# X-PLUG/Youku-mPLUG

Hardware: NVIDIA H100
Metric: video-text samples/sec (pretrain 1.3B, 8f x 224^2) (higher is better)
Workload: dtype bf16

## Files before the change

youku-mplug_b200/csrc/attention.cu:

```cuda
#include <math_constants.h>
#include <stdlib.h>

#include "common.h"
#include "philox.cuh"
#include "ptx.cuh"
#include "wgmma.cuh"

namespace ymp {

struct SeqMap {
  int seq_div, n_prefix, prefix_per_seq;
  long outer_stride, inner_stride, pos_stride, prefix_base, prefix_stride;
};
static SeqMap to_map(const ymp_seqmap& m) {
  SeqMap r;
  r.seq_div = m.seq_div > 0 ? m.seq_div : 1;
  r.n_prefix = m.n_prefix; r.prefix_per_seq = m.prefix_per_seq;
  r.outer_stride = m.outer_stride; r.inner_stride = m.inner_stride; r.pos_stride = m.pos_stride;
  r.prefix_base = m.prefix_base; r.prefix_stride = m.prefix_stride;
  return r;
}
struct RSeq {
  long base, pos_stride, prefix0;
  int n_prefix;
// ... 72 lines not shown
  a = w0 >= ds.thresh ? a * ds.scale : 0.f;
  b = w1 >= ds.thresh ? b * ds.scale : 0.f;
}
__device__ __forceinline__ float drop1(const DropState& ds, uint32_t row, uint32_t col, float a) {
  const uint4 w = drop_words(ds, row, col >> 2);
  const uint32_t c = col & 3, wc = c == 0 ? w.x : c == 1 ? w.y : c == 2 ? w.z : w.w;
  return wc >= ds.thresh ? a * ds.scale : 0.f;
}

__device__ __forceinline__ void eff_len(const AttnKParams& p, int s, int& sq, int& skv) {
  sq = p.s_q; skv = p.s_kv;
  if (p.skv_dev) skv = min(skv, *p.skv_dev);
  if (p.total_rows > 0) {
    const long left = p.total_rows - (long)s * p.s_q;
    if (left < sq) sq = (int)left;
    if (left < skv) skv = (int)left;
  }
}
__device__ __forceinline__ bool tile_needs_mask(const AttnKParams& p, int row_lo, int col0, int skv) {
  if (col0 + 64 > skv) return true;
  if (p.mask == MASK_CAUSAL) return col0 + 63 > row_lo;
  return p.mask == MASK_BLOCK;
}
__device__ __forceinline__ void apply_mask(const AttnKParams& p, float (&sc)[8][4], int row_lo, int col0, int skv,
                                           int g, int t4, float fill) {
  const int r0 = row_lo + g, r1 = r0 + 8;
  int rb0 = 0, rb1 = 0;
  if (p.mask == MASK_BLOCK) { rb0 = r0 / p.mask_block; rb1 = r1 / p.mask_block; }
#pragma unroll
  for (int nb = 0; nb < 8; ++nb) {
#pragma unroll
    for (int e = 0; e < 2; ++e) {
      const int col = col0 + nb * 8 + t4 * 2 + e;
      bool m0 = col >= skv, m1 = m0;
      if (p.mask == MASK_CAUSAL) { m0 |= col > r0; m1 |= col > r1; }
      else if (p.mask == MASK_BLOCK) { const int cb = col / p.mask_block; m0 |= cb != rb0; m1 |= cb != rb1; }
      if (m0) sc[nb][e] = fill;
      if (m1) sc[nb][2 + e] = fill;
    }
  }
}
template <bool BLOCK>
__device__ __forceinline__ void apply_mask_t(const AttnKParams& p, float (&st)[8][4], int k_lo, int qi0, int skv, int g,
                                             int t4) {
  bool need = k_lo + 16 > skv;
  if (p.mask == MASK_CAUSAL) need |= k_lo + 15 > qi0;
  if (BLOCK && p.mask == MASK_BLOCK) need = true;
  if (!need) return;
  const int k0 = k_lo + g, k1 = k0 + 8;
  int kb0 = 0, kb1 = 0;
  if (BLOCK && p.mask == MASK_BLOCK) { kb0 = k0 / p.mask_block; kb1 = k1 / p.mask_block; }
#pragma unroll
  for (int nb = 0; nb < 8; ++nb) {
#pragma unroll
    for (int e = 0; e < 2; ++e) {
      const int qc = qi0 + nb * 8 + t4 * 2 + e;
      bool m0 = k0 >= skv, m1 = k1 >= skv;
      if (p.mask == MASK_CAUSAL) { m0 |= k0 > qc; m1 |= k1 > qc; }
      else if (BLOCK && p.mask == MASK_BLOCK) { const int qb = qc / p.mask_block; m0 |= qb != kb0; m1 |= qb != kb1; }
      if (m0) st[nb][e] = -CUDART_INF_F;
      if (m1) st[nb][2 + e] = -CUDART_INF_F;
    }
  }
}

template <bool BLOCK>
__device__ __forceinline__ int key_tiles(const AttnKParams& p, int a_lo, int sq, int skv, int& kv_begin) {
  int kv_end = skv;
  kv_begin = 0;
  if (p.mask == MASK_CAUSAL) kv_end = min(skv, a_lo + 64);
  if (BLOCK && p.mask == MASK_BLOCK) {
    kv_begin = (a_lo / p.mask_block) * p.mask_block / 64 * 64;
    kv_end = min(skv, ((min(a_lo + 64, sq) - 1) / p.mask_block + 1) * p.mask_block);
  }
  return (kv_end - kv_begin + 63) / 64;
}
__device__ __forceinline__ void warp_key_span(const AttnKParams& p, int r_lo, int kv0, int skv, int& nv, int& nb_lo) {
  nv = min(64, skv - kv0);
  nb_lo = 0;
  if (p.mask == MASK_CAUSAL) nv = min(nv, r_lo + 16 - kv0);
  if (p.mask == MASK_BLOCK) {
    const int c_lo = (r_lo / p.mask_block) * p.mask_block, c_hi = ((r_lo + 15) / p.mask_block + 1) * p.mask_block;
    nb_lo = max(0, (c_lo - kv0) / 16);
    nv = min(nv, c_hi - kv0);
  }
}

template <int ND>
__device__ __forceinline__ void softmax_step(const AttnKParams& p, float (&sc)[8][4], float (&m_i)[2], float (&l_i)[2],
                                             float (&o_acc)[ND][4]) {
  float mx[2] = {-CUDART_INF_F, -CUDART_INF_F};
#pragma unroll
  for (int nb = 0; nb < 8; ++nb) {
    mx[0] = fmaxf(mx[0], fmaxf(sc[nb][0], sc[nb][1]));
    mx[1] = fmaxf(mx[1], fmaxf(sc[nb][2], sc[nb][3]));
  }
  float alpha[2], ms[2];
#pragma unroll
  for (int r = 0; r < 2; ++r) {
    mx[r] = fmaxf(mx[r], __shfl_xor_sync(0xffffffffu, mx[r], 1));
    mx[r] = fmaxf(mx[r], __shfl_xor_sync(0xffffffffu, mx[r], 2));
    const float mnew = fmaxf(m_i[r], mx[r]);
    ms[r] = (mnew == -CUDART_INF_F) ? 0.f : mnew * p.scale_log2;
    alpha[r] = exp2f(m_i[r] * p.scale_log2 - ms[r]);
    m_i[r] = mnew;
    l_i[r] *= alpha[r];
  }
#pragma unroll
  for (int nb = 0; nb < 8; ++nb) {
#pragma unroll
    for (int e = 0; e < 4; ++e) {
      const float pv = exp2f(fmaf(sc[nb][e], p.scale_log2, -ms[e >> 1]));
      sc[nb][e] = pv;
      l_i[e >> 1] += pv;
    }
  }
#pragma unroll
  for (int i = 0; i < ND; ++i) {
    o_acc[i][0] *= alpha[0]; o_acc[i][1] *= alpha[0];
    o_acc[i][2] *= alpha[1]; o_acc[i][3] *= alpha[1];
  }
}
__device__ __forceinline__ void drop_tile(const DropState& ds, uint32_t drow0, int kv0, int t4, float (&f)[8][4]) {
#pragma unroll
  for (int nb = 0; nb < 8; ++nb) {
    const uint32_t col = (uint32_t)(kv0 + nb * 8 + t4 * 2);
    drop2(ds, drow0, col, f[nb][0], f[nb][1]);
    drop2(ds, drow0 + 8, col, f[nb][2], f[nb][3]);
  }
}
__device__ __forceinline__ void scores_to_ds(const AttnKParams& p, float (&sc)[8][4], const float (&dp)[8][4],
                                             const float (&lse_r)[2], const float (&del_r)[2]) {
#pragma unroll
  for (int nb = 0; nb < 8; ++nb) {
#pragma unroll
    for (int e = 0; e < 4; ++e) {
      const float pv = exp2f(fmaf(sc[nb][e], p.scale_log2, -lse_r[e >> 1]));
      sc[nb][e] = pv * (dp[nb][e] - del_r[e >> 1]);
    }
  }
}
template <bool QUAD_EXCHANGE>
__device__ __forceinline__ void probs_t(const AttnKParams& p, const DropState& ds, float (&st)[8][4], float (&dpt)[8][4],
                                        const float* stat, uint32_t qrow0, int k_lo, int lane) {
  const int g = lane >> 2, t4 = lane & 3;
#pragma unroll
  for (int nb = 0; nb < 8; ++nb) {
    uint32_t keep = 0xFu;
    if (QUAD_EXCHANGE && p.has_drop) {
      const int j = g & 3;
      const uint32_t qr = qrow0 + (uint32_t)(nb * 8 + t4 * 2 + (j & 1));
      const uint4 w = drop_words(ds, qr, (uint32_t)(k_lo + (g & ~3) + (j >> 1) * 8) >> 2);
      keep = 0;
#pragma unroll
      for (int r = 0; r < 4; ++r) {
        const int comp = (j + r) & 3, c = (j - r) & 3;
        const uint32_t v = comp == 0 ? w.x : comp == 1 ? w.y : comp == 2 ? w.z : w.w;
        const uint32_t got = __shfl_sync(0xffffffffu, v, (lane & ~0xC) | (c << 2));
        keep |= (got >= ds.thresh ? 1u : 0u) << c;
      }
    }
#pragma unroll
    for (int e = 0; e < 4; ++e) {
      const int ql = nb * 8 + t4 * 2 + (e & 1);
      const float pv = exp2f(fmaf(st[nb][e], p.scale_log2, -stat[ql]));
      float dz = dpt[nb][e];
      if (p.has_drop) {
        float kf;
        if constexpr (QUAD_EXCHANGE) {
          kf = (keep >> e) & 1u ? ds.scale : 0.f;
// ... 460 lines not shown
      }
    }
    __syncthreads();
  }
  if (!warp_active) return;
  store_dkdv<D, DIO>(p, dk_acc, dv_acc, kv0 + warp * 16, skv, h, mdkv, g, t4);
}

template <int D>
struct WgTile {
  static constexpr int BYTES = ((D + 63) / 64) * 8192;
};
__device__ __forceinline__ uint64_t wg_desc_k(uint32_t base, int ks) {
  return make_smem_desc(base + (ks >> 2) * 8192 + (ks & 3) * 32, 16, 1024, 1);
}
__device__ __forceinline__ uint64_t wg_desc_mn(uint32_t base, int ks) { return make_smem_desc(base + ks * 2048, 8192, 1024, 1); }

template <int D>
__device__ __forceinline__ void wg_rs(float (&d)[D / 2], const uint32_t (&a)[4], uint64_t db) {
  if constexpr (D == 64) wgmma_rs_m64n64_tb(d, a, db);
  else if constexpr (D == 80) wgmma_rs_m64n80_tb(d, a, db);
  else wgmma_rs_m64n96_tb(d, a, db);
}
template <int D>
__device__ __forceinline__ void wg_scores(float (&s)[8][4], uint32_t a, uint32_t b) {
  float (&f)[32] = *reinterpret_cast<float(*)[32]>(&s[0][0]);
#pragma unroll
  for (int i = 0; i < 32; ++i) f[i] = 0.f;
  wgmma_fence_acc(f);
  wgmma_fence();
#pragma unroll
  for (int kk = 0; kk < D / 16; ++kk) wgmma_ss_m64n64(f, wg_desc_k(a, kk), wg_desc_k(b, kk));
  wgmma_commit();
  wgmma_wait<0>();
  wgmma_fence_acc(f);
}
template <int D>
__device__ __forceinline__ void wg_pv(float (&acc)[D / 8][4], const float (&pm)[8][4], uint32_t t) {
  float (&f)[D / 2] = *reinterpret_cast<float(*)[D / 2]>(&acc[0][0]);
  uint32_t pa[4][4];
#pragma unroll
  for (int kk = 0; kk < 4; ++kk) {
    pa[kk][0] = pack_bf16(pm[2 * kk][0], pm[2 * kk][1]);
    pa[kk][1] = pack_bf16(pm[2 * kk][2], pm[2 * kk][3]);
    pa[kk][2] = pack_bf16(pm[2 * kk + 1][0], pm[2 * kk + 1][1]);
    pa[kk][3] = pack_bf16(pm[2 * kk + 1][2], pm[2 * kk + 1][3]);
  }
  wgmma_fence_acc(f);
  wgmma_fence();
#pragma unroll
  for (int kk = 0; kk < 4; ++kk) wg_rs<D>(f, pa[kk], wg_desc_mn(t, kk));
  wgmma_commit();
  wgmma_wait<0>();
  wgmma_fence_acc(f);
}

template <bool CACHE>
__device__ __forceinline__ auto with_cache(const RMat& m, const __nv_bfloat16* c, const AttnKParams& p, int s, int h) {
  if constexpr (CACHE) return RMatC{m, c + (long)(s / p.mkv.seq_div) * p.n0 * p.ldc + h * p.hsc, p.ldc, p.n0};
  else return m;
}

template <bool PACKED>
__device__ __forceinline__ RSeq seq_rows(const SeqMap& m, int s, int r0) {
  if constexpr (PACKED) return RSeq{r0, 1, 0, 0};
  else return resolve(m, s);
}

template <int D, int DIO, bool TABLE = false, bool CACHE = false, bool PACKED = false>
__global__ void __launch_bounds__(128) attn_wg_fwd_kernel(const AttnKParams p) {
  constexpr int TB = WgTile<D>::BYTES;
  extern __shared__ uint8_t smem_wg[];
  uint8_t* sm = smem_wg + ((1024u - (smem_u32(smem_wg) & 1023u)) & 1023u);
  uint8_t* Qs = sm;
  uint8_t* KVs = sm + TB;
  const int warp = threadIdx.x >> 5, lane = threadIdx.x & 31;
  const int h = blockIdx.y, s = blockIdx.z;
  const int g = lane >> 2, t4 = lane & 3;
  int qoff = p.mask == MASK_CAUSAL ? p.s_kv - p.s_q : 0;
  int q0 = blockIdx.x * 64 - (qoff & 63), a0 = q0 + qoff;
  if constexpr (TABLE) {
    qoff = __ldg(p.n_prefix + s / p.mkv.seq_div);
    q0 = blockIdx.x * 64 - (qoff & 63);
    a0 = q0 + qoff;
  }
  int sq, skv;
  eff_len(p, s, sq, skv);
  if constexpr (TABLE) skv = qoff + sq;
  int r0 = 0;
  if constexpr (PACKED) {
    r0 = __ldg(p.starts + s);
    sq = skv = __ldg(p.starts + s + 1) - r0;
  }
  if (q0 >= sq) return;
  RSeq mkv = seq_rows<PACKED>(p.mkv, s, r0);
  const RSeq mo = seq_rows<PACKED>(p.mo, s, r0);
  if constexpr (TABLE) mkv.n_prefix = CACHE ? qoff - p.n0 : qoff;
  const RMat Mq = rmat(p.q, seq_rows<PACKED>(p.mq, s, r0), p.ldq, h * p.hsq);
  const auto Mk = with_cache<CACHE>(rmat(p.k, mkv, p.ldk, h * p.hsk), p.kc, p, s, h);
  const auto Mv = with_cache<CACHE>(rmat(p.v, mkv, p.ldv, h * p.hsv), p.vc, p, s, h);
  int kv_begin;
  const int ntiles = key_tiles<false>(p, a0, sq, skv, kv_begin);

  load_tile<SWIZZLE_128B, D, DIO>(Qs, Mq, q0, sq);
  load_tile<SWIZZLE_128B, D, DIO>(KVs, Mk, kv_begin, skv);
  load_tile<SWIZZLE_128B, D, DIO>(KVs + TB, Mv, kv_begin, skv);
  cp_async_commit();

  float o_acc[D / 8][4];
#pragma unroll
  for (int i = 0; i < D / 8; ++i) { o_acc[i][0] = o_acc[i][1] = o_acc[i][2] = o_acc[i][3] = 0.f; }
  float m_i[2] = {-CUDART_INF_F, -CUDART_INF_F}, l_i[2] = {0.f, 0.f};
  DropState ds;
  if (p.has_drop) ds = drop_state(p.drop);
  const uint32_t drow0 = (uint32_t)(((long)s * p.n_heads + h) * p.s_q + q0 + warp * 16 + g);

  for (int t = 0; t < ntiles; ++t) {
    const int kv0 = kv_begin + t * 64;
    uint8_t* Ks = KVs + (t & 1) * 2 * TB;
    uint8_t* Vs = Ks + TB;
    if (t + 1 < ntiles) {
      uint8_t* Kn = KVs + ((t + 1) & 1) * 2 * TB;
      load_tile<SWIZZLE_128B, D, DIO>(Kn, Mk, kv0 + 64, skv);
      load_tile<SWIZZLE_128B, D, DIO>(Kn + TB, Mv, kv0 + 64, skv);
      cp_async_commit();
      cp_async_wait<1>();
    } else {
      cp_async_wait<0>();
    }
    fence_proxy_async();
    __syncthreads();
    float sc[8][4];
    wg_scores<D>(sc, smem_u32(Qs), smem_u32(Ks));
    if (tile_needs_mask(p, a0 + warp * 16, kv0, skv)) apply_mask(p, sc, a0 + warp * 16, kv0, skv, g, t4, -CUDART_INF_F);
    softmax_step(p, sc, m_i, l_i, o_acc);
    if (p.has_drop) drop_tile(ds, drow0, kv0, t4, sc);
    wg_pv<D>(o_acc, sc, smem_u32(Vs));
    __syncthreads();
  }
  store_o_lse<D, DIO, PACKED>(p, o_acc, m_i, l_i, q0 + warp * 16, sq, s, h, mo, g, t4);
}

template <int D, int DIO>
__global__ void __launch_bounds__(128) attn_wg_bwd_dq_kernel(const AttnKParams p) {
  constexpr int TB = WgTile<D>::BYTES;
  extern __shared__ uint8_t smem_wg[];
  uint8_t* sm = smem_wg + ((1024u - (smem_u32(smem_wg) & 1023u)) & 1023u);
  uint8_t* Qs = sm;
  uint8_t* dOs = sm + TB;
  uint8_t* KVs = sm + 2 * TB;
  float* stat = reinterpret_cast<float*>(sm + 6 * TB);
  const int warp = threadIdx.x >> 5, lane = threadIdx.x & 31;
  const int q0 = blockIdx.x * 64, h = blockIdx.y, s = blockIdx.z;
  const int g = lane >> 2, t4 = lane & 3;
  int sq, skv;
  eff_len(p, s, sq, skv);
  if (q0 >= sq) return;
  const RSeq mkv = resolve(p.mkv, s), mo = resolve(p.mo, s), mdo = resolve(p.mdo, s), mdq = resolve(p.mdq, s);
  const RMat Mq = rmat(p.q, resolve(p.mq, s), p.ldq, h * p.hsq), Mdo = rmat(p.dout, mdo, p.lddo, h * p.hsdo);
  const RMat Mk = rmat(p.k, mkv, p.ldk, h * p.hsk), Mv = rmat(p.v, mkv, p.ldv, h * p.hsv);
  int kv_begin;
  const int ntiles = key_tiles<false>(p, q0, sq, skv, kv_begin);

  load_tile<SWIZZLE_128B, D, DIO>(Qs, Mq, q0, sq);
  load_tile<SWIZZLE_128B, D, DIO>(dOs, Mdo, q0, sq);
  load_tile<SWIZZLE_128B, D, DIO>(KVs, Mk, kv_begin, skv);
  load_tile<SWIZZLE_128B, D, DIO>(KVs + TB, Mv, kv_begin, skv);
  cp_async_commit();
  stage_dq_stats<DIO>(p, s, h, q0 + warp * 16, sq, mo, mdo, stat + warp * 16);
  float dq_acc[D / 8][4];
#pragma unroll
  for (int i = 0; i < D / 8; ++i) { dq_acc[i][0] = dq_acc[i][1] = dq_acc[i][2] = dq_acc[i][3] = 0.f; }
  float lse_r[2], del_r[2];
  DropState ds;
  if (p.has_drop) ds = drop_state(p.drop);
  const uint32_t drow0 = (uint32_t)(((long)s * p.n_heads + h) * p.s_q + q0 + warp * 16 + g);

  for (int t = 0; t < ntiles; ++t) {
    const int kv0 = kv_begin + t * 64;
    uint8_t* Ks = KVs + (t & 1) * 2 * TB;
    uint8_t* Vs = Ks + TB;
    if (t + 1 < ntiles) {
      uint8_t* Kn = KVs + ((t + 1) & 1) * 2 * TB;
      load_tile<SWIZZLE_128B, D, DIO>(Kn, Mk, kv0 + 64, skv);
      load_tile<SWIZZLE_128B, D, DIO>(Kn + TB, Mv, kv0 + 64, skv);
      cp_async_commit();
      cp_async_wait<1>();
    } else {
      cp_async_wait<0>();
    }
    fence_proxy_async();
    __syncthreads();
    if (t == 0) {
      lse_r[0] = stat[warp * 16 + g]; lse_r[1] = stat[warp * 16 + g + 8];
      del_r[0] = stat[64 + warp * 16 + g]; del_r[1] = stat[64 + warp * 16 + g + 8];
    }
    float sc[8][4], dp[8][4];
    wg_scores<D>(sc, smem_u32(Qs), smem_u32(Ks));
    wg_scores<D>(dp, smem_u32(dOs), smem_u32(Vs));
    if (tile_needs_mask(p, q0 + warp * 16, kv0, skv)) apply_mask(p, sc, q0 + warp * 16, kv0, skv, g, t4, -CUDART_INF_F);
    if (p.has_drop) drop_tile(ds, drow0, kv0, t4, dp);
    scores_to_ds(p, sc, dp, lse_r, del_r);
    wg_pv<D>(dq_acc, sc, smem_u32(Ks));
    __syncthreads();
  }
  store_dq<D, DIO>(p, dq_acc, q0 + warp * 16, sq, h, mdq, g, t4);
}

template <int D, int DIO>
__global__ void __launch_bounds__(128) attn_wg_bwd_dkdv_kernel(const AttnKParams p) {
  constexpr int TB = WgTile<D>::BYTES;
  extern __shared__ uint8_t smem_wg[];
  uint8_t* sm = smem_wg + ((1024u - (smem_u32(smem_wg) & 1023u)) & 1023u);
  uint8_t* Ks = sm;
  uint8_t* Vs = sm + TB;
  uint8_t* QDs = sm + 2 * TB;
  float* stat = reinterpret_cast<float*>(sm + 6 * TB);
  const int warp = threadIdx.x >> 5, lane = threadIdx.x & 31;
  const int kv0 = blockIdx.x * 64, h = blockIdx.y, s = blockIdx.z;
  const int g = lane >> 2, t4 = lane & 3;
  int sq, skv;
  eff_len(p, s, sq, skv);
  if (kv0 >= skv) return;
  const RSeq mkv = resolve(p.mkv, s), mdkv = resolve(p.mdkv, s);
  const RMat Mq = rmat(p.q, resolve(p.mq, s), p.ldq, h * p.hsq), Mdo = rmat(p.dout, resolve(p.mdo, s), p.lddo, h * p.hsdo);
  const RMat Mk = rmat(p.k, mkv, p.ldk, h * p.hsk), Mv = rmat(p.v, mkv, p.ldv, h * p.hsv);
  const int q_begin = (p.mask == MASK_CAUSAL) ? kv0 : 0;
  const int ntiles = (sq - q_begin + 63) / 64;
// ... 1 lines not shown

  auto load_stage = [&](int stage, int qi0) {
    uint8_t* Qn = QDs + stage * 2 * TB;
    load_tile<SWIZZLE_128B, D, DIO>(Qn, Mq, qi0, sq);
    load_tile<SWIZZLE_128B, D, DIO>(Qn + TB, Mdo, qi0, sq);
    stage_dkdv_stats(p, stat_base, qi0, sq, stat + stage * 128);
  };

  load_tile<SWIZZLE_128B, D, DIO>(Ks, Mk, kv0, skv);
  load_tile<SWIZZLE_128B, D, DIO>(Vs, Mv, kv0, skv);
  load_stage(0, q_begin);
  cp_async_commit();

  float dk_acc[D / 8][4], dv_acc[D / 8][4];
#pragma unroll
  for (int i = 0; i < D / 8; ++i) {
    dk_acc[i][0] = dk_acc[i][1] = dk_acc[i][2] = dk_acc[i][3] = 0.f;
    dv_acc[i][0] = dv_acc[i][1] = dv_acc[i][2] = dv_acc[i][3] = 0.f;
  }
  DropState ds;
  if (p.has_drop) ds = drop_state(p.drop);
  const uint32_t dbase = (uint32_t)stat_base;

  for (int t = 0; t < ntiles; ++t) {
    const int qi0 = q_begin + t * 64;
    uint8_t* Qs = QDs + (t & 1) * 2 * TB;
    uint8_t* dOs = Qs + TB;
    const float* st = stat + (t & 1) * 128;
    if (t + 1 < ntiles) {
      load_stage((t + 1) & 1, qi0 + 64);
      cp_async_commit();
      cp_async_wait<1>();
    } else {
      cp_async_wait<0>();
    }
    fence_proxy_async();
    __syncthreads();
    float st_[8][4], dpt[8][4];
    wg_scores<D>(st_, smem_u32(Ks), smem_u32(Qs));
    wg_scores<D>(dpt, smem_u32(Vs), smem_u32(dOs));
    apply_mask_t<false>(p, st_, kv0 + warp * 16, qi0, skv, g, t4);
    probs_t<true>(p, ds, st_, dpt, st, dbase + (uint32_t)qi0, kv0 + warp * 16, lane);
    wg_pv<D>(dv_acc, st_, smem_u32(dOs));
    wg_pv<D>(dk_acc, dpt, smem_u32(Qs));
    __syncthreads();
  }
  store_dkdv<D, DIO>(p, dk_acc, dv_acc, kv0 + warp * 16, skv, h, mdkv, g, t4);
}

template <int D, bool SEQ_LENS>
__device__ __forceinline__ void attn_decode(const AttnKParams& p) {
  constexpr int CH = D / 8;
  extern __shared__ __align__(16) uint8_t smem_attn[];
  float (*o_part)[D + 1] = reinterpret_cast<float (*)[D + 1]>(smem_attn);
  float* l_part = reinterpret_cast<float*>(smem_attn) + 128 * (D + 1);
  float* m_part = l_part + 128;
  const int lane = threadIdx.x & 31, warp = threadIdx.x >> 5;
  const int h = blockIdx.x, s = blockIdx.y;
  const int* table = p.kv_rows ? p.kv_rows + s * p.kv_rows_ld : nullptr;
  const RSeq mkv = table ? RSeq{0, 1, 0, 0} : resolve(p.mkv, s);
  const RMat Mk = rmat(p.k, mkv, p.ldk, h * p.hsk), Mv = rmat(p.v, mkv, p.ldv, h * p.hsv);
  const __nv_bfloat16* qrow = p.q + rrow(resolve(p.mq, s), 0) * p.ldq + h * p.hsq;
  constexpr bool TWO_PHASE = D > 80;
  uint4 qv[CH], kv[CH], vv[CH];
#pragma unroll
  for (int c = 0; c < CH; ++c) qv[c] = __ldg(reinterpret_cast<const uint4*>(qrow) + c);
  auto row_of = [&](int key) { return table ? __ldg(table + key) : key; };
  auto fetch_k = [&](int row) {
    const uint4* kr = reinterpret_cast<const uint4*>(mrow(Mk, row));
// ... 126 lines not shown
}
template <void (*K)(AttnKParams)>
static int launch_attn(dim3 grid, int smem, cudaStream_t st, const AttnKParams& p) {
  static DeviceOnce once;
  if (once.first()) { YMP_CUDA(cudaFuncSetAttribute(K, cudaFuncAttributeMaxDynamicSharedMemorySize, smem)); }
  K<<<grid, 128, smem, st>>>(p);
  YMP_LAUNCH_CHECK();
  return YMP_OK;
}

template <bool SEQ_LENS = false>
static int launch_decode(const AttnKParams& p, int head_dim, cudaStream_t st) {
  return for_head_dim<false>(head_dim, [&](auto hd) {
    constexpr int D = decltype(hd)::D;
    constexpr auto kernel = SEQ_LENS ? attn_decode_lens_kernel<D> : attn_decode_kernel<D>;
    return launch_attn<kernel>(dim3(p.n_heads, p.n_seq), (128 * (D + 1) + 128 + 4) * 4, st, p);
  });
}
static int launch_wg_fwd(const AttnKParams& p, int head_dim, cudaStream_t st) {
  const int lead = p.mask == MASK_CAUSAL ? (p.s_kv - p.s_q) & 63 : 0;
  const dim3 grid((p.s_q + lead + 63) / 64, p.n_heads, p.n_seq);
  return for_head_dim<false>(head_dim, [&](auto hd) {
    using H = decltype(hd);
    return launch_attn<attn_wg_fwd_kernel<H::D, H::DIO>>(grid, 5 * WgTile<H::D>::BYTES + 1024, st, p);
  });
}
template <bool CACHE>
static int launch_wg_fwd_table(const AttnKParams& p, int head_dim, cudaStream_t st) {
  const dim3 grid((p.s_q + 126) / 64, p.n_heads, p.n_seq);
  return for_head_dim<false>(head_dim, [&](auto hd) {
    using H = decltype(hd);
    return launch_attn<attn_wg_fwd_kernel<H::D, H::DIO, true, CACHE>>(grid, 5 * WgTile<H::D>::BYTES + 1024, st, p);
  });
}
static int launch_wg_fwd_packed(const AttnKParams& p, int head_dim, cudaStream_t st) {
  const dim3 grid((p.s_q + 63) / 64, p.n_heads, p.n_seq);
  return for_head_dim<false>(head_dim, [&](auto hd) {
    using H = decltype(hd);
    return launch_attn<attn_wg_fwd_kernel<H::D, H::DIO, false, false, true>>(grid, 5 * WgTile<H::D>::BYTES + 1024, st, p);
  });
}
static int launch_wg_bwd(const AttnKParams& p, int head_dim, cudaStream_t st) {
  return for_head_dim<false>(head_dim, [&](auto hd) {
    using H = decltype(hd);
    const int smem = 6 * WgTile<H::D>::BYTES + 1024 + 1024;
    const int rc = launch_attn<attn_wg_bwd_dq_kernel<H::D, H::DIO>>(dim3((p.s_q + 63) / 64, p.n_heads, p.n_seq), smem, st, p);
    if (rc) return rc;
    return launch_attn<attn_wg_bwd_dkdv_kernel<H::D, H::DIO>>(dim3((p.s_kv + 63) / 64, p.n_heads, p.n_seq), smem, st, p);
  });
}
static int launch_fwd(const AttnKParams& p, int head_dim, cudaStream_t st) {
  return for_head_dim<true>(head_dim, [&](auto hd) {
    using H = decltype(hd);
    return launch_attn<attn_fwd_kernel<H::D, H::DIO>>(dim3((p.s_q + 63) / 64, p.n_heads, p.n_seq), 5 * 64 * (H::D + 8) * 2, st, p);
  });
}
static int launch_bwd(const AttnKParams& p, int head_dim, cudaStream_t st) {
  return for_head_dim<true>(head_dim, [&](auto hd) {
    using H = decltype(hd);
    const int smem = 6 * 64 * (H::D + 8) * 2 + 1024;
    const int rc = launch_attn<attn_bwd_dq_kernel<H::D, H::DIO>>(dim3((p.s_q + 63) / 64, p.n_heads, p.n_seq), smem, st, p);
    if (rc) return rc;
// ... 169 lines not shown
```

youku-mplug_b200/csrc/wgmma.cuh:

```cuda
#pragma once
#include <stdint.h>

namespace ymp {

template <int TA, int TB>
__device__ __forceinline__ void wgmma_m64n256(float (&d)[128], uint64_t da, uint64_t db, uint32_t scale_d) {
  asm volatile(
      "{\n\t.reg .pred p;\n\t"
      "setp.ne.b32 p, %130, 0;\n\t"
      "wgmma.mma_async.sync.aligned.m64n256k16.f32.bf16.bf16 {%0, %1, %2, %3, %4, %5, %6, %7, %8, %9, %10, %11, %12, %13, %14, %15, %16, %17, %18, %19, %20, %21, %22, %23, %24, %25, %26, %27, %28, %29, %30, %31, %32, %33, %34, %35, %36, %37, %38, %39, %40, %41, %42, %43, %44, %45, %46, %47, %48, %49, %50, %51, %52, %53, %54, %55, %56, %57, %58, %59, %60, %61, %62, %63, %64, %65, %66, %67, %68, %69, %70, %71, %72, %73, %74, %75, %76, %77, %78, %79, %80, %81, %82, %83, %84, %85, %86, %87, %88, %89, %90, %91, %92, %93, %94, %95, %96, %97, %98, %99, %100, %101, %102, %103, %104, %105, %106, %107, %108, %109, %110, %111, %112, %113, %114, %115, %116, %117, %118, %119, %120, %121, %122, %123, %124, %125, %126, %127}, %128, %129, p, 1, 1, %131, %132;\n\t}\n"
      : "+f"(d[0]), "+f"(d[1]), "+f"(d[2]), "+f"(d[3]), "+f"(d[4]), "+f"(d[5]), "+f"(d[6]), "+f"(d[7]), "+f"(d[8]), "+f"(d[9]), "+f"(d[10]), "+f"(d[11]), "+f"(d[12]), "+f"(d[13]), "+f"(d[14]), "+f"(d[15]), "+f"(d[16]), "+f"(d[17]), "+f"(d[18]), "+f"(d[19]), "+f"(d[20]), "+f"(d[21]), "+f"(d[22]), "+f"(d[23]), "+f"(d[24]), "+f"(d[25]), "+f"(d[26]), "+f"(d[27]), "+f"(d[28]), "+f"(d[29]), "+f"(d[30]), "+f"(d[31]), "+f"(d[32]), "+f"(d[33]), "+f"(d[34]), "+f"(d[35]), "+f"(d[36]), "+f"(d[37]), "+f"(d[38]), "+f"(d[39]), "+f"(d[40]), "+f"(d[41]), "+f"(d[42]), "+f"(d[43]), "+f"(d[44]), "+f"(d[45]), "+f"(d[46]), "+f"(d[47]), "+f"(d[48]), "+f"(d[49]), "+f"(d[50]), "+f"(d[51]), "+f"(d[52]), "+f"(d[53]), "+f"(d[54]), "+f"(d[55]), "+f"(d[56]), "+f"(d[57]), "+f"(d[58]), "+f"(d[59]), "+f"(d[60]), "+f"(d[61]), "+f"(d[62]), "+f"(d[63]), "+f"(d[64]), "+f"(d[65]), "+f"(d[66]), "+f"(d[67]), "+f"(d[68]), "+f"(d[69]), "+f"(d[70]), "+f"(d[71]), "+f"(d[72]), "+f"(d[73]), "+f"(d[74]), "+f"(d[75]), "+f"(d[76]), "+f"(d[77]), "+f"(d[78]), "+f"(d[79]), "+f"(d[80]), "+f"(d[81]), "+f"(d[82]), "+f"(d[83]), "+f"(d[84]), "+f"(d[85]), "+f"(d[86]), "+f"(d[87]), "+f"(d[88]), "+f"(d[89]), "+f"(d[90]), "+f"(d[91]), "+f"(d[92]), "+f"(d[93]), "+f"(d[94]), "+f"(d[95]), "+f"(d[96]), "+f"(d[97]), "+f"(d[98]), "+f"(d[99]), "+f"(d[100]), "+f"(d[101]), "+f"(d[102]), "+f"(d[103]), "+f"(d[104]), "+f"(d[105]), "+f"(d[106]), "+f"(d[107]), "+f"(d[108]), "+f"(d[109]), "+f"(d[110]), "+f"(d[111]), "+f"(d[112]), "+f"(d[113]), "+f"(d[114]), "+f"(d[115]), "+f"(d[116]), "+f"(d[117]), "+f"(d[118]), "+f"(d[119]), "+f"(d[120]), "+f"(d[121]), "+f"(d[122]), "+f"(d[123]), "+f"(d[124]), "+f"(d[125]), "+f"(d[126]), "+f"(d[127])
      : "l"(da), "l"(db), "r"(scale_d), "n"(TA), "n"(TB));
}

template <int TA, int TB>
__device__ __forceinline__ void wgmma_m64n128(float (&d)[64], uint64_t da, uint64_t db, uint32_t scale_d) {
  asm volatile(
      "{\n\t.reg .pred p;\n\t"
      "setp.ne.b32 p, %66, 0;\n\t"
      "wgmma.mma_async.sync.aligned.m64n128k16.f32.bf16.bf16 {%0, %1, %2, %3, %4, %5, %6, %7, %8, %9, %10, %11, %12, %13, %14, %15, %16, %17, %18, %19, %20, %21, %22, %23, %24, %25, %26, %27, %28, %29, %30, %31, %32, %33, %34, %35, %36, %37, %38, %39, %40, %41, %42, %43, %44, %45, %46, %47, %48, %49, %50, %51, %52, %53, %54, %55, %56, %57, %58, %59, %60, %61, %62, %63}, %64, %65, p, 1, 1, %67, %68;\n\t}\n"
      : "+f"(d[0]), "+f"(d[1]), "+f"(d[2]), "+f"(d[3]), "+f"(d[4]), "+f"(d[5]), "+f"(d[6]), "+f"(d[7]), "+f"(d[8]), "+f"(d[9]), "+f"(d[10]), "+f"(d[11]), "+f"(d[12]), "+f"(d[13]), "+f"(d[14]), "+f"(d[15]), "+f"(d[16]), "+f"(d[17]), "+f"(d[18]), "+f"(d[19]), "+f"(d[20]), "+f"(d[21]), "+f"(d[22]), "+f"(d[23]), "+f"(d[24]), "+f"(d[25]), "+f"(d[26]), "+f"(d[27]), "+f"(d[28]), "+f"(d[29]), "+f"(d[30]), "+f"(d[31]), "+f"(d[32]), "+f"(d[33]), "+f"(d[34]), "+f"(d[35]), "+f"(d[36]), "+f"(d[37]), "+f"(d[38]), "+f"(d[39]), "+f"(d[40]), "+f"(d[41]), "+f"(d[42]), "+f"(d[43]), "+f"(d[44]), "+f"(d[45]), "+f"(d[46]), "+f"(d[47]), "+f"(d[48]), "+f"(d[49]), "+f"(d[50]), "+f"(d[51]), "+f"(d[52]), "+f"(d[53]), "+f"(d[54]), "+f"(d[55]), "+f"(d[56]), "+f"(d[57]), "+f"(d[58]), "+f"(d[59]), "+f"(d[60]), "+f"(d[61]), "+f"(d[62]), "+f"(d[63])
      : "l"(da), "l"(db), "r"(scale_d), "n"(TA), "n"(TB));
}

__device__ __forceinline__ void wgmma_ss_m64n64(float (&d)[32], uint64_t da, uint64_t db) {
  asm volatile(
      "wgmma.mma_async.sync.aligned.m64n64k16.f32.bf16.bf16 {%0, %1, %2, %3, %4, %5, %6, %7, %8, %9, %10, %11, %12, %13, %14, %15, %16, %17, %18, %19, %20, %21, %22, %23, %24, %25, %26, %27, %28, %29, %30, %31}, %32, %33, 1, 1, 1, 0, 0;\n"
      : "+f"(d[0]), "+f"(d[1]), "+f"(d[2]), "+f"(d[3]), "+f"(d[4]), "+f"(d[5]), "+f"(d[6]), "+f"(d[7]), "+f"(d[8]), "+f"(d[9]), "+f"(d[10]), "+f"(d[11]), "+f"(d[12]), "+f"(d[13]), "+f"(d[14]), "+f"(d[15]), "+f"(d[16]), "+f"(d[17]), "+f"(d[18]), "+f"(d[19]), "+f"(d[20]), "+f"(d[21]), "+f"(d[22]), "+f"(d[23]), "+f"(d[24]), "+f"(d[25]), "+f"(d[26]), "+f"(d[27]), "+f"(d[28]), "+f"(d[29]), "+f"(d[30]), "+f"(d[31])
      : "l"(da), "l"(db));
}

__device__ __forceinline__ void wgmma_rs_m64n64_tb(float (&d)[32], const uint32_t (&a)[4], uint64_t db) {
  asm volatile(
      "wgmma.mma_async.sync.aligned.m64n64k16.f32.bf16.bf16 {%0, %1, %2, %3, %4, %5, %6, %7, %8, %9, %10, %11, %12, %13, %14, %15, %16, %17, %18, %19, %20, %21, %22, %23, %24, %25, %26, %27, %28, %29, %30, %31}, {%32, %33, %34, %35}, %36, 1, 1, 1, 1;\n"
      : "+f"(d[0]), "+f"(d[1]), "+f"(d[2]), "+f"(d[3]), "+f"(d[4]), "+f"(d[5]), "+f"(d[6]), "+f"(d[7]), "+f"(d[8]), "+f"(d[9]), "+f"(d[10]), "+f"(d[11]), "+f"(d[12]), "+f"(d[13]), "+f"(d[14]), "+f"(d[15]), "+f"(d[16]), "+f"(d[17]), "+f"(d[18]), "+f"(d[19]), "+f"(d[20]), "+f"(d[21]), "+f"(d[22]), "+f"(d[23]), "+f"(d[24]), "+f"(d[25]), "+f"(d[26]), "+f"(d[27]), "+f"(d[28]), "+f"(d[29]), "+f"(d[30]), "+f"(d[31])
      : "r"(a[0]), "r"(a[1]), "r"(a[2]), "r"(a[3]), "l"(db));
}

__device__ __forceinline__ void wgmma_rs_m64n80_tb(float (&d)[40], const uint32_t (&a)[4], uint64_t db) {
  asm volatile(
      "wgmma.mma_async.sync.aligned.m64n80k16.f32.bf16.bf16 {%0, %1, %2, %3, %4, %5, %6, %7, %8, %9, %10, %11, %12, %13, %14, %15, %16, %17, %18, %19, %20, %21, %22, %23, %24, %25, %26, %27, %28, %29, %30, %31, %32, %33, %34, %35, %36, %37, %38, %39}, {%40, %41, %42, %43}, %44, 1, 1, 1, 1;\n"
      : "+f"(d[0]), "+f"(d[1]), "+f"(d[2]), "+f"(d[3]), "+f"(d[4]), "+f"(d[5]), "+f"(d[6]), "+f"(d[7]), "+f"(d[8]), "+f"(d[9]), "+f"(d[10]), "+f"(d[11]), "+f"(d[12]), "+f"(d[13]), "+f"(d[14]), "+f"(d[15]), "+f"(d[16]), "+f"(d[17]), "+f"(d[18]), "+f"(d[19]), "+f"(d[20]), "+f"(d[21]), "+f"(d[22]), "+f"(d[23]), "+f"(d[24]), "+f"(d[25]), "+f"(d[26]), "+f"(d[27]), "+f"(d[28]), "+f"(d[29]), "+f"(d[30]), "+f"(d[31]), "+f"(d[32]), "+f"(d[33]), "+f"(d[34]), "+f"(d[35]), "+f"(d[36]), "+f"(d[37]), "+f"(d[38]), "+f"(d[39])
      : "r"(a[0]), "r"(a[1]), "r"(a[2]), "r"(a[3]), "l"(db));
}

// ... 9 lines not shown
```

Measured before the change: 170.7.

## Trim tail key tiles to live width, batch wgmma pairs, rebalance fwd K/V smem staging

The last partial key/query tile in the forward and both backward WGMMA attention kernels now uses narrower wgmma shapes (n16/32/48), selected at compile time from the remaining live width, so padded columns are not computed. The two score GEMMs in the backward kernels are issued under one commit/wait, and the dV/dK updates are merged the same way, to reduce wgmma serialization. The forward kernel splits K and V staging so that for D>64 only one V buffer is kept, cutting shared memory, with extra waits and barriers to overlap the next K load. In exchange this instantiates more template variants (larger code, more registers) and makes the pipeline logic more intricate.

```diff
diff --git a/youku-mplug_b200/csrc/attention.cu b/youku-mplug_b200/csrc/attention.cu
--- a/youku-mplug_b200/csrc/attention.cu
+++ b/youku-mplug_b200/csrc/attention.cu
@@ -1,5 +1,6 @@
 #include <math_constants.h>
 #include <stdlib.h>
+#include <type_traits>
 
 #include "common.h"
 #include "philox.cuh"
@@ -118,13 +119,14 @@
   if (p.mask == MASK_CAUSAL) return col0 + 63 > row_lo;
   return p.mask == MASK_BLOCK;
 }
+template <int NB = 8>
 __device__ __forceinline__ void apply_mask(const AttnKParams& p, float (&sc)[8][4], int row_lo, int col0, int skv,
                                            int g, int t4, float fill) {
   const int r0 = row_lo + g, r1 = r0 + 8;
   int rb0 = 0, rb1 = 0;
   if (p.mask == MASK_BLOCK) { rb0 = r0 / p.mask_block; rb1 = r1 / p.mask_block; }
 #pragma unroll
-  for (int nb = 0; nb < 8; ++nb) {
+  for (int nb = 0; nb < NB; ++nb) {
 #pragma unroll
     for (int e = 0; e < 2; ++e) {
       const int col = col0 + nb * 8 + t4 * 2 + e;
@@ -136,7 +138,7 @@
     }
   }
 }
-template <bool BLOCK>
+template <bool BLOCK, int NB = 8>
 __device__ __forceinline__ void apply_mask_t(const AttnKParams& p, float (&st)[8][4], int k_lo, int qi0, int skv, int g,
                                              int t4) {
   bool need = k_lo + 16 > skv;
@@ -147,7 +149,7 @@
   int kb0 = 0, kb1 = 0;
   if (BLOCK && p.mask == MASK_BLOCK) { kb0 = k0 / p.mask_block; kb1 = k1 / p.mask_block; }
 #pragma unroll
-  for (int nb = 0; nb < 8; ++nb) {
+  for (int nb = 0; nb < NB; ++nb) {
 #pragma unroll
     for (int e = 0; e < 2; ++e) {
       const int qc = qi0 + nb * 8 + t4 * 2 + e;
@@ -182,12 +184,12 @@
   }
 }
 
-template <int ND>
+template <int ND, int NB = 8>
 __device__ __forceinline__ void softmax_step(const AttnKParams& p, float (&sc)[8][4], float (&m_i)[2], float (&l_i)[2],
                                              float (&o_acc)[ND][4]) {
   float mx[2] = {-CUDART_INF_F, -CUDART_INF_F};
 #pragma unroll
-  for (int nb = 0; nb < 8; ++nb) {
+  for (int nb = 0; nb < NB; ++nb) {
     mx[0] = fmaxf(mx[0], fmaxf(sc[nb][0], sc[nb][1]));
     mx[1] = fmaxf(mx[1], fmaxf(sc[nb][2], sc[nb][3]));
   }
@@ -203,7 +205,7 @@
     l_i[r] *= alpha[r];
   }
 #pragma unroll
-  for (int nb = 0; nb < 8; ++nb) {
+  for (int nb = 0; nb < NB; ++nb) {
 #pragma unroll
     for (int e = 0; e < 4; ++e) {
       const float pv = exp2f(fmaf(sc[nb][e], p.scale_log2, -ms[e >> 1]));
@@ -217,18 +219,20 @@
     o_acc[i][2] *= alpha[1]; o_acc[i][3] *= alpha[1];
   }
 }
+template <int NB = 8>
 __device__ __forceinline__ void drop_tile(const DropState& ds, uint32_t drow0, int kv0, int t4, float (&f)[8][4]) {
 #pragma unroll
-  for (int nb = 0; nb < 8; ++nb) {
+  for (int nb = 0; nb < NB; ++nb) {
     const uint32_t col = (uint32_t)(kv0 + nb * 8 + t4 * 2);
     drop2(ds, drow0, col, f[nb][0], f[nb][1]);
     drop2(ds, drow0 + 8, col, f[nb][2], f[nb][3]);
   }
 }
+template <int NB = 8>
 __device__ __forceinline__ void scores_to_ds(const AttnKParams& p, float (&sc)[8][4], const float (&dp)[8][4],
                                              const float (&lse_r)[2], const float (&del_r)[2]) {
 #pragma unroll
-  for (int nb = 0; nb < 8; ++nb) {
+  for (int nb = 0; nb < NB; ++nb) {
 #pragma unroll
     for (int e = 0; e < 4; ++e) {
       const float pv = exp2f(fmaf(sc[nb][e], p.scale_log2, -lse_r[e >> 1]));
@@ -236,12 +240,12 @@
     }
   }
 }
-template <bool QUAD_EXCHANGE>
+template <bool QUAD_EXCHANGE, int NB = 8>
 __device__ __forceinline__ void probs_t(const AttnKParams& p, const DropState& ds, float (&st)[8][4], float (&dpt)[8][4],
                                         const float* stat, uint32_t qrow0, int k_lo, int lane) {
   const int g = lane >> 2, t4 = lane & 3;
 #pragma unroll
-  for (int nb = 0; nb < 8; ++nb) {
+  for (int nb = 0; nb < NB; ++nb) {
     uint32_t keep = 0xFu;
     if (QUAD_EXCHANGE && p.has_drop) {
       const int j = g & 3;
@@ -748,37 +752,102 @@
   else if constexpr (D == 80) wgmma_rs_m64n80_tb(d, a, db);
   else wgmma_rs_m64n96_tb(d, a, db);
 }
-template <int D>
+template <int D, int NB>
+__device__ __forceinline__ void wg_scores_mma(float (&f)[NB * 4], uint32_t a, uint32_t b) {
+#pragma unroll
+  for (int kk = 0; kk < D / 16; ++kk) {
+    if constexpr (NB == 2) wgmma_ss_m64n16(f, wg_desc_k(a, kk), wg_desc_k(b, kk));
+    else if constexpr (NB == 4) wgmma_ss_m64n32(f, wg_desc_k(a, kk), wg_desc_k(b, kk));
+    else if constexpr (NB == 6) wgmma_ss_m64n48(f, wg_desc_k(a, kk), wg_desc_k(b, kk));
+    else wgmma_ss_m64n64(f, wg_desc_k(a, kk), wg_desc_k(b, kk));
+  }
+}
+template <int NB>
+__device__ __forceinline__ float (&wg_frag(float (&s)[8][4]))[NB * 4] {
+  return *reinterpret_cast<float(*)[NB * 4]>(&s[0][0]);
+}
+template <int D, int NB = 8>
 __device__ __forceinline__ void wg_scores(float (&s)[8][4], uint32_t a, uint32_t b) {
-  float (&f)[32] = *reinterpret_cast<float(*)[32]>(&s[0][0]);
-#pragma unroll
-  for (int i = 0; i < 32; ++i) f[i] = 0.f;
+  float (&f)[NB * 4] = wg_frag<NB>(s);
+#pragma unroll
+  for (int i = 0; i < NB * 4; ++i) f[i] = 0.f;
   wgmma_fence_acc(f);
   wgmma_fence();
-#pragma unroll
-  for (int kk = 0; kk < D / 16; ++kk) wgmma_ss_m64n64(f, wg_desc_k(a, kk), wg_desc_k(b, kk));
+  wg_scores_mma<D, NB>(f, a, b);
   wgmma_commit();
   wgmma_wait<0>();
   wgmma_fence_acc(f);
 }
-template <int D>
-__device__ __forceinline__ void wg_pv(float (&acc)[D / 8][4], const float (&pm)[8][4], uint32_t t) {
-  float (&f)[D / 2] = *reinterpret_cast<float(*)[D / 2]>(&acc[0][0]);
-  uint32_t pa[4][4];
-#pragma unroll
-  for (int kk = 0; kk < 4; ++kk) {
+template <int D, int NB = 8>
+__device__ __forceinline__ void wg_scores2(float (&s1)[8][4], uint32_t a1, uint32_t b1, float (&s2)[8][4], uint32_t a2,
+                                           uint32_t b2) {
+  float (&f1)[NB * 4] = wg_frag<NB>(s1);
+  float (&f2)[NB * 4] = wg_frag<NB>(s2);
+#pragma unroll
+  for (int i = 0; i < NB * 4; ++i) f1[i] = f2[i] = 0.f;
+  wgmma_fence_acc(f1);
+  wgmma_fence_acc(f2);
+  wgmma_fence();
+  wg_scores_mma<D, NB>(f1, a1, b1);
+  wg_scores_mma<D, NB>(f2, a2, b2);
+  wgmma_commit();
+  wgmma_wait<0>();
+  wgmma_fence_acc(f1);
+  wgmma_fence_acc(f2);
+}
+template <int NB>
+__device__ __forceinline__ void wg_pack(uint32_t (&pa)[NB / 2][4], const float (&pm)[8][4]) {
+#pragma unroll
+  for (int kk = 0; kk < NB / 2; ++kk) {
     pa[kk][0] = pack_bf16(pm[2 * kk][0], pm[2 * kk][1]);
     pa[kk][1] = pack_bf16(pm[2 * kk][2], pm[2 * kk][3]);
     pa[kk][2] = pack_bf16(pm[2 * kk + 1][0], pm[2 * kk + 1][1]);
     pa[kk][3] = pack_bf16(pm[2 * kk + 1][2], pm[2 * kk + 1][3]);
   }
+}
+template <int D, int NB = 8>
+__device__ __forceinline__ void wg_pv(float (&acc)[D / 8][4], const float (&pm)[8][4], uint32_t t) {
+  float (&f)[D / 2] = *reinterpret_cast<float(*)[D / 2]>(&acc[0][0]);
+  uint32_t pa[NB / 2][4];
+  wg_pack<NB>(pa, pm);
   wgmma_fence_acc(f);
   wgmma_fence();
 #pragma unroll
-  for (int kk = 0; kk < 4; ++kk) wg_rs<D>(f, pa[kk], wg_desc_mn(t, kk));
+  for (int kk = 0; kk < NB / 2; ++kk) wg_rs<D>(f, pa[kk], wg_desc_mn(t, kk));
   wgmma_commit();
   wgmma_wait<0>();
   wgmma_fence_acc(f);
+}
+template <int D, int NB = 8>
+__device__ __forceinline__ void wg_pv2(float (&acc1)[D / 8][4], const float (&pm1)[8][4], uint32_t t1,
+                                       float (&acc2)[D / 8][4], const float (&pm2)[8][4], uint32_t t2) {
+  float (&f1)[D / 2] = *reinterpret_cast<float(*)[D / 2]>(&acc1[0][0]);
+  float (&f2)[D / 2] = *reinterpret_cast<float(*)[D / 2]>(&acc2[0][0]);
+  uint32_t pa1[NB / 2][4], pa2[NB / 2][4];
+  wg_pack<NB>(pa1, pm1);
+  wg_pack<NB>(pa2, pm2);
+  wgmma_fence_acc(f1);
+  wgmma_fence_acc(f2);
+  wgmma_fence();
+#pragma unroll
+  for (int kk = 0; kk < NB / 2; ++kk) wg_rs<D>(f1, pa1[kk], wg_desc_mn(t1, kk));
+#pragma unroll
+  for (int kk = 0; kk < NB / 2; ++kk) wg_rs<D>(f2, pa2[kk], wg_desc_mn(t2, kk));
+  wgmma_commit();
+  wgmma_wait<0>();
+  wgmma_fence_acc(f1);
+  wgmma_fence_acc(f2);
+}
+template <class F>
+__device__ __forceinline__ void with_live_width(int w, F&& f) {
+  if (w > 48) f(std::integral_constant<int, 8>{});
+  else if (w > 32) f(std::integral_constant<int, 6>{});
+  else if (w > 16) f(std::integral_constant<int, 4>{});
+  else f(std::integral_constant<int, 2>{});
+}
+__device__ __forceinline__ int full_tiles(int n, int ntiles) { return n < 64 * ntiles ? ntiles - 1 : ntiles; }
+__device__ __forceinline__ int key_end(const AttnKParams& p, int a_lo, int skv) {
+  return p.mask == MASK_CAUSAL ? min(skv, a_lo + 64) : skv;
 }
 
 template <bool CACHE>
@@ -793,13 +862,20 @@
   else return resolve(m, s);
 }
 
+template <int D>
+struct WgFwdSmem {
+  static constexpr int V_STAGES = D == 64 ? 2 : 1;
+  static constexpr int BYTES = (3 + V_STAGES) * WgTile<D>::BYTES + 1024;
+};
 template <int D, int DIO, bool TABLE = false, bool CACHE = false, bool PACKED = false>
 __global__ void __launch_bounds__(128) attn_wg_fwd_kernel(const AttnKParams p) {
   constexpr int TB = WgTile<D>::BYTES;
   extern __shared__ uint8_t smem_wg[];
   uint8_t* sm = smem_wg + ((1024u - (smem_u32(smem_wg) & 1023u)) & 1023u);
+  constexpr int VS = WgFwdSmem<D>::V_STAGES;
   uint8_t* Qs = sm;
-  uint8_t* KVs = sm + TB;
+  uint8_t* Kr = sm + TB;
+  uint8_t* Vr = sm + 3 * TB;
   const int warp = threadIdx.x >> 5, lane = threadIdx.x & 31;
   const int h = blockIdx.y, s = blockIdx.z;
   const int g = lane >> 2, t4 = lane & 3;
@@ -826,11 +902,12 @@
   const auto Mk = with_cache<CACHE>(rmat(p.k, mkv, p.ldk, h * p.hsk), p.kc, p, s, h);
   const auto Mv = with_cache<CACHE>(rmat(p.v, mkv, p.ldv, h * p.hsv), p.vc, p, s, h);
   int kv_begin;
-  const int ntiles = key_tiles<false>(p, a0, sq, skv, kv_begin);
+  const int ntiles = key_tiles<false>(p, a0, sq, skv, kv_begin), kv_end = key_end(p, a0, skv);
 
   load_tile<SWIZZLE_128B, D, DIO>(Qs, Mq, q0, sq);
-  load_tile<SWIZZLE_128B, D, DIO>(KVs, Mk, kv_begin, skv);
-  load_tile<SWIZZLE_128B, D, DIO>(KVs + TB, Mv, kv_begin, skv);
+  load_tile<SWIZZLE_128B, D, DIO>(Kr, Mk, kv_begin, skv);
+  if constexpr (VS == 1) cp_async_commit();
+  load_tile<SWIZZLE_128B, D, DIO>(Vr, Mv, kv_begin, skv);
   cp_async_commit();
 
   float o_acc[D / 8][4];
@@ -841,29 +918,45 @@
   if (p.has_drop) ds = drop_state(p.drop);
   const uint32_t drow0 = (uint32_t)(((long)s * p.n_heads + h) * p.s_q + q0 + warp * 16 + g);
 
-  for (int t = 0; t < ntiles; ++t) {
+  auto tile = [&](int t, auto nb) {
+    constexpr int NB = decltype(nb)::value;
     const int kv0 = kv_begin + t * 64;
-    uint8_t* Ks = KVs + (t & 1) * 2 * TB;
-    uint8_t* Vs = Ks + TB;
-    if (t + 1 < ntiles) {
-      uint8_t* Kn = KVs + ((t + 1) & 1) * 2 * TB;
-      load_tile<SWIZZLE_128B, D, DIO>(Kn, Mk, kv0 + 64, skv);
-      load_tile<SWIZZLE_128B, D, DIO>(Kn + TB, Mv, kv0 + 64, skv);
+    uint8_t* Ks = Kr + (t & 1) * TB;
+    uint8_t* Vs = Vr + (VS == 2 ? (t & 1) * TB : 0);
+    if constexpr (VS == 2) {
+      if (t + 1 < ntiles) {
+        load_tile<SWIZZLE_128B, D, DIO>(Kr + ((t + 1) & 1) * TB, Mk, kv0 + 64, skv);
+        load_tile<SWIZZLE_128B, D, DIO>(Vr + ((t + 1) & 1) * TB, Mv, kv0 + 64, skv);
+      }
       cp_async_commit();
       cp_async_wait<1>();
     } else {
-      cp_async_wait<0>();
+      if (t + 1 < ntiles) load_tile<SWIZZLE_128B, D, DIO>(Kr + ((t + 1) & 1) * TB, Mk, kv0 + 64, skv);
+      cp_async_commit();
+      cp_async_wait<2>();
     }
     fence_proxy_async();
     __syncthreads();
     float sc[8][4];
-    wg_scores<D>(sc, smem_u32(Qs), smem_u32(Ks));
-    if (tile_needs_mask(p, a0 + warp * 16, kv0, skv)) apply_mask(p, sc, a0 + warp * 16, kv0, skv, g, t4, -CUDART_INF_F);
-    softmax_step(p, sc, m_i, l_i, o_acc);
-    if (p.has_drop) drop_tile(ds, drow0, kv0, t4, sc);
-    wg_pv<D>(o_acc, sc, smem_u32(Vs));
+    wg_scores<D, NB>(sc, smem_u32(Qs), smem_u32(Ks));
+    if (tile_needs_mask(p, a0 + warp * 16, kv0, skv)) apply_mask<NB>(p, sc, a0 + warp * 16, kv0, skv, g, t4, -CUDART_INF_F);
+    softmax_step<D / 8, NB>(p, sc, m_i, l_i, o_acc);
+    if (p.has_drop) drop_tile<NB>(ds, drow0, kv0, t4, sc);
+    if constexpr (VS == 1) {
+      cp_async_wait<1>();
+      fence_proxy_async();
+      __syncthreads();
+    }
+    wg_pv<D, NB>(o_acc, sc, smem_u32(Vs));
     __syncthreads();
-  }
+    if constexpr (VS == 1) {
+      if (t + 1 < ntiles) load_tile<SWIZZLE_128B, D, DIO>(Vr, Mv, kv0 + 64, skv);
+      cp_async_commit();
+    }
+  };
+  const int nfull = DIO == D ? full_tiles(kv_end - kv_begin, ntiles) : ntiles;
+  for (int t = 0; t < nfull; ++t) tile(t, std::integral_constant<int, 8>{});
+  if (nfull < ntiles) with_live_width(kv_end - kv_begin - 64 * nfull, [&](auto nb) { tile(nfull, nb); });
   store_o_lse<D, DIO, PACKED>(p, o_acc, m_i, l_i, q0 + warp * 16, sq, s, h, mo, g, t4);
 }
 
@@ -886,7 +979,7 @@
   const RMat Mq = rmat(p.q, resolve(p.mq, s), p.ldq, h * p.hsq), Mdo = rmat(p.dout, mdo, p.lddo, h * p.hsdo);
   const RMat Mk = rmat(p.k, mkv, p.ldk, h * p.hsk), Mv = rmat(p.v, mkv, p.ldv, h * p.hsv);
   int kv_begin;
-  const int ntiles = key_tiles<false>(p, q0, sq, skv, kv_begin);
+  const int ntiles = key_tiles<false>(p, q0, sq, skv, kv_begin), kv_end = key_end(p, q0, skv);
 
   load_tile<SWIZZLE_128B, D, DIO>(Qs, Mq, q0, sq);
   load_tile<SWIZZLE_128B, D, DIO>(dOs, Mdo, q0, sq);
@@ -902,7 +995,8 @@
   if (p.has_drop) ds = drop_state(p.drop);
   const uint32_t drow0 = (uint32_t)(((long)s * p.n_heads + h) * p.s_q + q0 + warp * 16 + g);
 
-  for (int t = 0; t < ntiles; ++t) {
+  auto tile = [&](int t, auto nb) {
+    constexpr int NB = decltype(nb)::value;
     const int kv0 = kv_begin + t * 64;
     uint8_t* Ks = KVs + (t & 1) * 2 * TB;
     uint8_t* Vs = Ks + TB;
@@ -922,14 +1016,16 @@
       del_r[0] = stat[64 + warp * 16 + g]; del_r[1] = stat[64 + warp * 16 + g + 8];
     }
     float sc[8][4], dp[8][4];
-    wg_scores<D>(sc, smem_u32(Qs), smem_u32(Ks));
-    wg_scores<D>(dp, smem_u32(dOs), smem_u32(Vs));
-    if (tile_needs_mask(p, q0 + warp * 16, kv0, skv)) apply_mask(p, sc, q0 + warp * 16, kv0, skv, g, t4, -CUDART_INF_F);
-    if (p.has_drop) drop_tile(ds, drow0, kv0, t4, dp);
-    scores_to_ds(p, sc, dp, lse_r, del_r);
-    wg_pv<D>(dq_acc, sc, smem_u32(Ks));
+    wg_scores2<D, NB>(sc, smem_u32(Qs), smem_u32(Ks), dp, smem_u32(dOs), smem_u32(Vs));
+    if (tile_needs_mask(p, q0 + warp * 16, kv0, skv)) apply_mask<NB>(p, sc, q0 + warp * 16, kv0, skv, g, t4, -CUDART_INF_F);
+    if (p.has_drop) drop_tile<NB>(ds, drow0, kv0, t4, dp);
+    scores_to_ds<NB>(p, sc, dp, lse_r, del_r);
+    wg_pv<D, NB>(dq_acc, sc, smem_u32(Ks));
     __syncthreads();
-  }
+  };
+  const int nfull = full_tiles(kv_end - kv_begin, ntiles);
+  for (int t = 0; t < nfull; ++t) tile(t, std::integral_constant<int, 8>{});
+  if (nfull < ntiles) with_live_width(kv_end - kv_begin - 64 * nfull, [&](auto nb) { tile(nfull, nb); });
   store_dq<D, DIO>(p, dq_acc, q0 + warp * 16, sq, h, mdq, g, t4);
 }
 
@@ -977,7 +1073,8 @@
   if (p.has_drop) ds = drop_state(p.drop);
   const uint32_t dbase = (uint32_t)stat_base;
 
-  for (int t = 0; t < ntiles; ++t) {
+  auto tile = [&](int t, auto nb) {
+    constexpr int NB = decltype(nb)::value;
     const int qi0 = q_begin + t * 64;
     uint8_t* Qs = QDs + (t & 1) * 2 * TB;
     uint8_t* dOs = Qs + TB;
@@ -992,14 +1089,15 @@
     fence_proxy_async();
     __syncthreads();
     float st_[8][4], dpt[8][4];
-    wg_scores<D>(st_, smem_u32(Ks), smem_u32(Qs));
-    wg_scores<D>(dpt, smem_u32(Vs), smem_u32(dOs));
-    apply_mask_t<false>(p, st_, kv0 + warp * 16, qi0, skv, g, t4);
-    probs_t<true>(p, ds, st_, dpt, st, dbase + (uint32_t)qi0, kv0 + warp * 16, lane);
-    wg_pv<D>(dv_acc, st_, smem_u32(dOs));
-    wg_pv<D>(dk_acc, dpt, smem_u32(Qs));
+    wg_scores2<D, NB>(st_, smem_u32(Ks), smem_u32(Qs), dpt, smem_u32(Vs), smem_u32(dOs));
+    apply_mask_t<false, NB>(p, st_, kv0 + warp * 16, qi0, skv, g, t4);
+    probs_t<true, NB>(p, ds, st_, dpt, st, dbase + (uint32_t)qi0, kv0 + warp * 16, lane);
+    wg_pv2<D, NB>(dv_acc, st_, smem_u32(dOs), dk_acc, dpt, smem_u32(Qs));
     __syncthreads();
-  }
+  };
+  const int nfull = full_tiles(sq - q_begin, ntiles);
+  for (int t = 0; t < nfull; ++t) tile(t, std::integral_constant<int, 8>{});
+  if (nfull < ntiles) with_live_width(sq - q_begin - 64 * nfull, [&](auto nb) { tile(nfull, nb); });
   store_dkdv<D, DIO>(p, dk_acc, dv_acc, kv0 + warp * 16, skv, h, mdkv, g, t4);
 }
 
@@ -1172,7 +1270,7 @@
   const dim3 grid((p.s_q + lead + 63) / 64, p.n_heads, p.n_seq);
   return for_head_dim<false>(head_dim, [&](auto hd) {
     using H = decltype(hd);
-    return launch_attn<attn_wg_fwd_kernel<H::D, H::DIO>>(grid, 5 * WgTile<H::D>::BYTES + 1024, st, p);
+    return launch_attn<attn_wg_fwd_kernel<H::D, H::DIO>>(grid, WgFwdSmem<H::D>::BYTES, st, p);
   });
 }
 template <bool CACHE>
@@ -1180,14 +1278,14 @@
   const dim3 grid((p.s_q + 126) / 64, p.n_heads, p.n_seq);
   return for_head_dim<false>(head_dim, [&](auto hd) {
     using H = decltype(hd);
-    return launch_attn<attn_wg_fwd_kernel<H::D, H::DIO, true, CACHE>>(grid, 5 * WgTile<H::D>::BYTES + 1024, st, p);
+    return launch_attn<attn_wg_fwd_kernel<H::D, H::DIO, true, CACHE>>(grid, WgFwdSmem<H::D>::BYTES, st, p);
   });
 }
 static int launch_wg_fwd_packed(const AttnKParams& p, int head_dim, cudaStream_t st) {
   const dim3 grid((p.s_q + 63) / 64, p.n_heads, p.n_seq);
   return for_head_dim<false>(head_dim, [&](auto hd) {
     using H = decltype(hd);
-    return launch_attn<attn_wg_fwd_kernel<H::D, H::DIO, false, false, true>>(grid, 5 * WgTile<H::D>::BYTES + 1024, st, p);
+    return launch_attn<attn_wg_fwd_kernel<H::D, H::DIO, false, false, true>>(grid, WgFwdSmem<H::D>::BYTES, st, p);
   });
 }
 static int launch_wg_bwd(const AttnKParams& p, int head_dim, cudaStream_t st) {
diff --git a/youku-mplug_b200/csrc/wgmma.cuh b/youku-mplug_b200/csrc/wgmma.cuh
--- a/youku-mplug_b200/csrc/wgmma.cuh
+++ b/youku-mplug_b200/csrc/wgmma.cuh
@@ -21,6 +21,27 @@
       "wgmma.mma_async.sync.aligned.m64n128k16.f32.bf16.bf16 {%0, %1, %2, %3, %4, %5, %6, %7, %8, %9, %10, %11, %12, %13, %14, %15, %16, %17, %18, %19, %20, %21, %22, %23, %24, %25, %26, %27, %28, %29, %30, %31, %32, %33, %34, %35, %36, %37, %38, %39, %40, %41, %42, %43, %44, %45, %46, %47, %48, %49, %50, %51, %52, %53, %54, %55, %56, %57, %58, %59, %60, %61, %62, %63}, %64, %65, p, 1, 1, %67, %68;\n\t}\n"
       : "+f"(d[0]), "+f"(d[1]), "+f"(d[2]), "+f"(d[3]), "+f"(d[4]), "+f"(d[5]), "+f"(d[6]), "+f"(d[7]), "+f"(d[8]), "+f"(d[9]), "+f"(d[10]), "+f"(d[11]), "+f"(d[12]), "+f"(d[13]), "+f"(d[14]), "+f"(d[15]), "+f"(d[16]), "+f"(d[17]), "+f"(d[18]), "+f"(d[19]), "+f"(d[20]), "+f"(d[21]), "+f"(d[22]), "+f"(d[23]), "+f"(d[24]), "+f"(d[25]), "+f"(d[26]), "+f"(d[27]), "+f"(d[28]), "+f"(d[29]), "+f"(d[30]), "+f"(d[31]), "+f"(d[32]), "+f"(d[33]), "+f"(d[34]), "+f"(d[35]), "+f"(d[36]), "+f"(d[37]), "+f"(d[38]), "+f"(d[39]), "+f"(d[40]), "+f"(d[41]), "+f"(d[42]), "+f"(d[43]), "+f"(d[44]), "+f"(d[45]), "+f"(d[46]), "+f"(d[47]), "+f"(d[48]), "+f"(d[49]), "+f"(d[50]), "+f"(d[51]), "+f"(d[52]), "+f"(d[53]), "+f"(d[54]), "+f"(d[55]), "+f"(d[56]), "+f"(d[57]), "+f"(d[58]), "+f"(d[59]), "+f"(d[60]), "+f"(d[61]), "+f"(d[62]), "+f"(d[63])
       : "l"(da), "l"(db), "r"(scale_d), "n"(TA), "n"(TB));
+}
+
+__device__ __forceinline__ void wgmma_ss_m64n16(float (&d)[8], uint64_t da, uint64_t db) {
+  asm volatile(
+      "wgmma.mma_async.sync.aligned.m64n16k16.f32.bf16.bf16 {%0, %1, %2, %3, %4, %5, %6, %7}, %8, %9, 1, 1, 1, 0, 0;\n"
+      : "+f"(d[0]), "+f"(d[1]), "+f"(d[2]), "+f"(d[3]), "+f"(d[4]), "+f"(d[5]), "+f"(d[6]), "+f"(d[7])
+      : "l"(da), "l"(db));
+}
+
+__device__ __forceinline__ void wgmma_ss_m64n32(float (&d)[16], uint64_t da, uint64_t db) {
+  asm volatile(
+      "wgmma.mma_async.sync.aligned.m64n32k16.f32.bf16.bf16 {%0, %1, %2, %3, %4, %5, %6, %7, %8, %9, %10, %11, %12, %13, %14, %15}, %16, %17, 1, 1, 1, 0, 0;\n"
+      : "+f"(d[0]), "+f"(d[1]), "+f"(d[2]), "+f"(d[3]), "+f"(d[4]), "+f"(d[5]), "+f"(d[6]), "+f"(d[7]), "+f"(d[8]), "+f"(d[9]), "+f"(d[10]), "+f"(d[11]), "+f"(d[12]), "+f"(d[13]), "+f"(d[14]), "+f"(d[15])
+      : "l"(da), "l"(db));
+}
+
+__device__ __forceinline__ void wgmma_ss_m64n48(float (&d)[24], uint64_t da, uint64_t db) {
+  asm volatile(
+      "wgmma.mma_async.sync.aligned.m64n48k16.f32.bf16.bf16 {%0, %1, %2, %3, %4, %5, %6, %7, %8, %9, %10, %11, %12, %13, %14, %15, %16, %17, %18, %19, %20, %21, %22, %23}, %24, %25, 1, 1, 1, 0, 0;\n"
+      : "+f"(d[0]), "+f"(d[1]), "+f"(d[2]), "+f"(d[3]), "+f"(d[4]), "+f"(d[5]), "+f"(d[6]), "+f"(d[7]), "+f"(d[8]), "+f"(d[9]), "+f"(d[10]), "+f"(d[11]), "+f"(d[12]), "+f"(d[13]), "+f"(d[14]), "+f"(d[15]), "+f"(d[16]), "+f"(d[17]), "+f"(d[18]), "+f"(d[19]), "+f"(d[20]), "+f"(d[21]), "+f"(d[22]), "+f"(d[23])
+      : "l"(da), "l"(db));
 }
 
 __device__ __forceinline__ void wgmma_ss_m64n64(float (&d)[32], uint64_t da, uint64_t db) {
```

New measurement: 171.9 (median of 6 runs). About the same (+0.7%).
